# MuMuJun97/semantic_slam_mapping

Hardware: AMD Instinct MI355X
Metric: frames/sec semantic-mapping, 640x480 RGB-D (higher is better)
Workload: dtype u8; 1 GPU; configs[1]: synthetic 640x480 RGB-D + precomputed 12-class masks, 1k frames per GPU, ORB 1000 kp/frame, 5 ref frames, leaf 0.10 m; frames_per_gpu=1000, frames_all_gpus=1000, batch_frames=250, matcher_halo_frames=0, parallelism=single GPU

## Files before the change

### semantic_slam_mapping_amd/csrc/kernels_orb.hip

```cpp
#include "ssm_internal.h"
#include "../../include/ssm/fast_quick_core.h"
#include <cstdlib>
#include <type_traits>
#include <algorithm>
#include <cstring>
#include <vector>

#define WAVE 64

template <bool VEC>
__global__ void gray_kernel(const uint8_t* __restrict__ img, int W, int H, int stride0, uint8_t* __restrict__ pyr, int pyr_bytes)
{
    const int quads = stride0 >> 2;
    const int q = blockIdx.x * blockDim.x + threadIdx.x;
    if (q >= quads * H) return;
    const int y = q / quads, x = (q - y * quads) << 2;
    const uint8_t* src = img + (size_t)blockIdx.y * W * H * 3 + ((size_t)y * W + x) * 3;
    uint8_t* dst = pyr + (size_t)blockIdx.y * pyr_bytes + (size_t)y * stride0 + x;
    uint32_t out = 0;
    if (x >= W) { *reinterpret_cast<uint32_t*>(dst) = 0; return; }
    if (VEC) {
        const uint32_t* s = reinterpret_cast<const uint32_t*>(src);
        uint32_t a = s[0], b = s[1], c = s[2];
        uint32_t p0 = ((a & 255) * 1868 + ((a >> 8) & 255) * 9617 + ((a >> 16) & 255) * 4899 + 8192) >> 14;
// ... 694 lines not shown
        const int w0 = wsum[0], w1 = wsum[1], w2 = wsum[2];
        n = w0 + w1 + w2 + wsum[3];
        int base = (int)(incl - cnt) + (wv > 0 ? w0 : 0) + (wv > 1 ? w1 : 0) + (wv > 2 ? w2 : 0);
        const uint32_t ent = ((uint32_t)(tid >> 2) << 8) | (uint32_t)(32 * (tid & 3));
        while (m) { list[base++] = (uint16_t)(ent + (uint32_t)__builtin_ctz(m)); m &= m - 1u; }
    }
    __syncthreads();
    const int ix0 = X0 - xs0, iw = X1 - X0, iy0 = Y0 - ys0, ih = Y1 - Y0;
    for (int e0 = 0; e0 < n; e0 += 512) {
        const int m = min(n - e0, 512), H = (m + 1) >> 1;
        const bool act = wv * 64 < H;
        bool ka = false, kb = false; int ia = 0, ib = 0;
        if (act) {
            const int ea = tid, eb = H + tid;
            ia = list[e0 + min(ea, m - 1)]; ib = list[e0 + min(eb, m - 1)];
            const int sya = ia >> 8, sxa = ia & 255, syb = ib >> 8, sxb = ib & 255;
            const uint32_t S2 = fast_S2(&px[(sya + 3) * FT_PW + sxa + 4], &px[(syb + 3) * FT_PW + sxb + 4], FT_PW);
            const int Sa = (int)(S2 & 0xFFFFu), Sb = (int)(S2 >> 16);
            if (ea < H) sc[(sya + 1) * FT_SST + sxa + 1] = (uint8_t)Sa;
            if (eb < m) sc[(syb + 1) * FT_SST + sxb + 1] = (uint8_t)Sb;
            ka = ea < H && Sa > min_th && (unsigned)(sxa - ix0) < (unsigned)iw && (unsigned)(sya - iy0) < (unsigned)ih;
            kb = eb < m && Sb > min_th && (unsigned)(sxb - ix0) < (unsigned)iw && (unsigned)(syb - iy0) < (unsigned)ih;
        }
        __syncthreads();
        if (act) {
            const unsigned long long ba = __ballot(ka), bb = __ballot(kb);
            const int ca = __popcll(ba), cb = __popcll(bb);
            if (ca + cb) {
                int base = 0;
                if (lane == 0) base = atomicAdd(&nsurv, ca + cb);
                base = __shfl(base, 0, 64);
                const unsigned long long below = (1ull << lane) - 1ull;
                if (ka) list[base + __popcll(ba & below)] = (uint16_t)ia;
                if (kb) list[base + ca + __popcll(bb & below)] = (uint16_t)ib;
            }
        }
    }
    __syncthreads();
    const int n2 = nsurv;
    cand_t* out = cand + (size_t)frame * g.cand_total + L.cand_off;
    int32_t* nc = ncand + frame * g.nlevels + l;
    for (int e0 = 0; e0 < n2; e0 += 256) {
        if (e0 + wv * 64 >= n2) continue;
        const int e = e0 + tid;
        bool keep = false; int S = 0, sx = 0, sy = 0;
        if (e < n2) {
            const int i = list[e]; sy = i >> 8; sx = i & 255;
            const uint8_t* q = &sc[(sy + 1) * FT_SST + sx + 1];
            S = q[0];
            const int cx = cellx[sx + 1], cy = celly[sy + 1];
            const bool xl = cellx[sx] == cx, xr = cellx[sx + 2] == cx, yu = celly[sy] == cy, yd = celly[sy + 2] == cy;
            int nb = 0;
            if (yu) { nb = max(nb, (int)q[-FT_SST]); if (xl) nb = max(nb, (int)q[-FT_SST-1]); if (xr) nb = max(nb, (int)q[-FT_SST+1]); }
            if (yd) { nb = max(nb, (int)q[FT_SST]);  if (xl) nb = max(nb, (int)q[FT_SST-1]);  if (xr) nb = max(nb, (int)q[FT_SST+1]); }
            if (xl) nb = max(nb, (int)q[-1]);
            if (xr) nb = max(nb, (int)q[1]);
            keep = nb < S;
        }
        const unsigned long long bal = __ballot(keep);
        if (bal) {
            int base = 0;
            if (lane == 0) base = atomicAdd(&nstage, __popcll(bal));
            base = __shfl(base, 0, 64);
            if (keep) {
                const int k = base + __popcll(bal & ((1ull << lane) - 1ull));
                const int gx = xs0 + sx, gy = ys0 + sy;
                const int cj = cellx[sx + 1], ci = celly[sy + 1];
                atomicMax(&lmax[((ci - cy0) & 7) * 8 + ((cj - cx0) & 7)], S);
                cand_t c;
                c.x = (uint32_t)(gx - L.minBX) | ((uint32_t)(gy - L.minBY) << 12) | ((uint32_t)(S - 1) << 24);
                c.y = ((uint32_t)(ci * L.nCols + cj) << 14) | ((uint32_t)(gy - L.minBY - ci * L.hCell) << 7) | (uint32_t)(gx - L.minBX - cj * L.wCell);
                if (k < stage_cap) stage[k] = c;
                else { const int kg = atomicAdd(nc, 1); if (kg < L.cand_cap) out[kg] = c; }
            }
        }
    }
    __syncthreads();
    const int ns = min(nstage, stage_cap);
    if (tid == 0 && ns) gbase = atomicAdd(nc, ns);
    __syncthreads();
    for (int k = tid; k < ns; k += 256) if (gbase + k < L.cand_cap) out[gbase + k] = stage[k];
    if (tid < 64 && lmax[tid] > 0) {
        const int ci = cy0 + (tid >> 3), cj = cx0 + (tid & 7);
        atomicMax(&cellmax[(size_t)frame * g.cells_total + L.cell_off + ci * L.nCols + cj], lmax[tid]);
    }
}
__global__ void __launch_bounds__(256, 8)
fast_kernel(const uint8_t* __restrict__ pyr, OrbGeom g, cand_t* __restrict__ cand, int32_t* __restrict__ ncand, int32_t* __restrict__ cellmax, int stage_cap, int nframes)
{
    const int frame = blockIdx.x, tile_id = blockIdx.y;
    if (frame >= nframes) return;
    fast_tile<1>(frame, tile_id, pyr, g, cand, ncand, cellmax, stage_cap);
}
__global__ void __launch_bounds__(256)
fast_need_kernel(OrbGeom g, const int32_t* __restrict__ cellmax, int nframes, int32_t* __restrict__ work)
{
    const int i = blockIdx.x * blockDim.x + threadIdx.x;
    const int frame = i % ((nframes + 7) & ~7), tile_id = i / ((nframes + 7) & ~7);
    bool need = false;
    if (frame < nframes && tile_id < g.ftiles_total) {
        int l = 0;
        while (l + 1 < g.nlevels && tile_id >= g.L[l+1].ftile_off) l++;
        const LevelGeom& L = g.L[l];
        const int t = tile_id - L.ftile_off;
        const int trow = L.ftiles_x == 1 ? t : (int)__umulhi((uint32_t)t, L.fmulTX);
        int X0, X1, Y0, Y1;
        ftile_rect(L, t - trow * L.ftiles_x, trow, X0, X1, Y0, Y1);
        const int cx0 = (int)__umulhi((uint32_t)(X0 - L.minBX - 3), L.mulW), cy0 = (int)__umulhi((uint32_t)(Y0 - L.minBY - 3), L.mulH);
        const int cx1 = min((int)__umulhi((uint32_t)(X1 - 1 - L.minBX - 3), L.mulW), L.nCols - 1), cy1 = min((int)__umulhi((uint32_t)(Y1 - 1 - L.minBY - 3), L.mulH), L.nRows - 1);
        const int32_t* cm = cellmax + (size_t)frame * g.cells_total + L.cell_off;
        for (int ci = cy0; ci <= cy1 && !need; ci++) for (int cj = cx0; cj <= cx1; cj++) if (cm[ci * L.nCols + cj] <= g.ini_th) { need = true; break; }
    }
    const unsigned long long bal = __ballot(need);
    if (bal) {
        const int lane = threadIdx.x & 63;
        int base = 0;
        if (lane == 0) base = atomicAdd(work - 1, __popcll(bal));
        base = __shfl(base, 0, 64);
        if (need) work[base + __popcll(bal & ((1ull << lane) - 1ull))] = (tile_id << 16) | frame;
    }
}
__global__ void __launch_bounds__(256)
fast_retry_kernel(const uint8_t* __restrict__ pyr, OrbGeom g, cand_t* __restrict__ cand, int32_t* __restrict__ ncand, int32_t* __restrict__ cellmax, int stage_cap,
                  const int32_t* __restrict__ work)
{
    const int nwork = work[-1];
    for (int i = blockIdx.x; i < nwork; i += gridDim.x) {
        const int item = work[i];
        fast_tile<2>(item & 65535, item >> 16, pyr, g, cand, ncand, cellmax, stage_cap);
        __syncthreads();
    }
}
size_t k_fast_cellmax_ints(int nframes, const OrbGeom& g) { return (size_t)nframes * (g.cells_total + g.ftiles_total) + 16; }
size_t k_fast_ncand_pad(int nframes, const OrbGeom& g) { return ((size_t)nframes * g.nlevels + 63) & ~(size_t)63; }
hipError_t k_fast(int n, const OrbGeom& g, const uint8_t* pyr, cand_t* cand, int32_t* ncand, int32_t* cellmax, hipStream_t s)
{
    hipError_t e;
    const ptrdiff_t gap = cellmax - ncand;
    if (gap >= (ptrdiff_t)n * g.nlevels && gap <= (ptrdiff_t)1 << 24) e = hipMemsetAsync(ncand, 0, sizeof(int32_t) * (((size_t)gap + (size_t)n * g.cells_total + 4 + 3) & ~(size_t)3), s);
    else { e = hipMemsetAsync(ncand, 0, sizeof(int32_t) * n * g.nlevels, s); if (e == hipSuccess) e = hipMemsetAsync(cellmax, 0, sizeof(int32_t) * ((size_t)n * g.cells_total + 4), s); }
    if (e != hipSuccess) return e;
    static const int stage_cap = [] { const char* e = getenv("SSM_FAST_STAGE_CAP"); const int v = e ? atoi(e) : FT_STAGE; return v < 0 ? 0 : (v > FT_STAGE ? FT_STAGE : v); }();
    int32_t* work = cellmax + (size_t)n * g.cells_total + 4;
    const int n8 = (n + 7) & ~7;
    fast_kernel<<<dim3(n8, g.ftiles_total), 256, 0, s>>>(pyr, g, cand, ncand, cellmax, stage_cap, n);
    fast_need_kernel<<<(n8 * g.ftiles_total + 255) / 256, 256, 0, s>>>(g, cellmax, n, work);
    const int pairs = n * g.ftiles_total;
    fast_retry_kernel<<<pairs < 4096 ? pairs : 4096, 256, 0, s>>>(pyr, g, cand, ncand, cellmax, stage_cap, work);
    return hipGetLastError();
}

struct QNode { short x0, y0, x1, y1; };
#define DROPPED 0xFFFF
#define OT_KCAP 2048
#define OT_T 256
#define OT_UN 4
__device__ __forceinline__ uint32_t block_excl_scan_u32(uint32_t v, uint32_t* sw, uint32_t& total)
{
    const uint32_t inc = wave_incl_scan_u32(v);
    const int lane = threadIdx.x & 63, w = threadIdx.x >> 6;
    if (lane == 63) sw[w] = inc;
    __syncthreads();
    uint32_t base = 0, tot = 0;
#pragma unroll
    for (int k = 0; k < OT_T / 64; k++) { const uint32_t x = sw[k]; tot += x; if (k < w) base += x; }
    __syncthreads();
    total = tot;
    return inc - v + base;
}
#ifdef SSM_OT_PROF
__device__ unsigned long long ot_prof[8][8];
#define OTP_T0 long long otp_ = clock64();
#define OTP(k) { const long long n_ = clock64(); if (threadIdx.x == 0) atomicAdd(&ot_prof[blockIdx.y & 7][k], (unsigned long long)(n_ - otp_)); otp_ = n_; }
#define OTP_CNT(k) { if (threadIdx.x == 0) atomicAdd(&ot_prof[blockIdx.y & 7][k], 1ull); }
#else
#define OTP_T0
#define OTP(k)
#define OTP_CNT(k)
#endif
template <int NODES>
__global__ void __launch_bounds__(OT_T, NODES == 256 ? 8 : 1)
octree_kernel(OrbGeom g, const cand_t* __restrict__ cand, const int32_t* __restrict__ ncand, const int32_t* __restrict__ cellmax,
              uint16_t* __restrict__ node_of, uint32_t* __restrict__ sel, int32_t* __restrict__ nsel, int32_t* __restrict__ status)
{
    __shared__ QNode    nd[2][NODES];
    __shared__ uint32_t cnt[2][NODES];
    __shared__ uint32_t sq[2][NODES];
    __shared__ __attribute__((aligned(8))) uint32_t cc[NODES][4];
    __shared__ short    newpos[NODES];
    __shared__ __attribute__((aligned(8))) short childpos[NODES][4];
    __shared__ short    order[NODES];
    unsigned long long* best = reinterpret_cast<unsigned long long*>(&cc[0][0]);
    __shared__ uint16_t lnof[OT_KCAP];
    __shared__ uint16_t cumn[NODES];
    __shared__ uint32_t sscan[OT_T / 64];
    __shared__ int sL, sFinish, sMode, sErr, sValid, sFirst;
    const int l = blockIdx.y, f = blockIdx.x, tid = threadIdx.x;
    OTP_T0
    const LevelGeom& L = g.L[l];
    const int N = L.nfeat;
    int nc = ncand[f * g.nlevels + l];
    if (nc > L.cand_cap) { nc = L.cand_cap; if (tid == 0) atomicOr(status, 1); }
    const cand_t* gkeys = cand + (size_t)f * g.cand_total + L.cand_off;
    uint16_t* gnof = node_of + (size_t)f * g.cand_total + L.cand_off;
    const bool in_lds = nc <= OT_KCAP;
    constexpr int KPT = OT_KCAP / OT_T;
    uint32_t kxr[KPT];
#pragma unroll
    for (int u = 0; u < KPT; u++) kxr[u] = 0u;
#define KEY(i) (gkeys[i])
#define KEYX(i) (gkeys[i].x)
#define NOF(i) (in_lds ? lnof[i] : gnof[i])
#define SETNOF(i, v) do { if (in_lds) lnof[i] = (uint16_t)(v); else gnof[i] = (uint16_t)(v); } while (0)
    uint32_t* out = sel + (size_t)f * g.sel_total + L.sel_off;
    if (nc == 0) { if (tid == 0) nsel[f * g.nlevels + l] = 0; return; }
    const int nIni = L.nIni; const float hX = L.hX;
    for (int i = tid; i < nIni; i += OT_T) {
        QNode q; q.x0 = (short)(int)(hX * (float)i); q.y0 = 0; q.x1 = (short)(int)(hX * (float)(i + 1)); q.y1 = (short)(L.maxBY - L.minBY);
        nd[0][i] = q; cnt[0][i] = 0; sq[0][i] = i;
    }
    if (tid == 0) { sErr = 0; sValid = 0; }
    __syncthreads();
    const int32_t* cm = cellmax + (size_t)f * g.cells_total + L.cell_off;
    int nvalid = 0;
    auto init_trip = [&](auto lds_tag, int i0, cand_t (&k)[OT_UN]) {
        constexpr bool in_lds = decltype(lds_tag)::value;
        int cmv[OT_UN];
#pragma unroll
        for (int u = 0; u < OT_UN; u++) { const int i = i0 + u * OT_T; k[u] = i < nc ? KEY(i) : make_uint2(0u, 0u); }
#pragma unroll
        for (int u = 0; u < OT_UN; u++) cmv[u] = i0 + u * OT_T < nc ? cm[k[u].y >> 14] : 0;
#pragma unroll
        for (int u = 0; u < OT_UN; u++) {
            const int i = i0 + u * OT_T;
            if (i >= nc) continue;
            const int S = (int)(k[u].x >> 24) + 1;
            const int th = cmv[u] > g.ini_th ? g.ini_th : g.min_th;
            if (S <= th) { SETNOF(i, DROPPED); continue; }
            const int x = k[u].x & 4095;
            int b = (int)((float)x / hX); b = min(b, nIni - 1);
            SETNOF(i, b); atomicAdd(&cnt[0][b], 1u); nvalid++;
        }
    };
    if (in_lds) {
#pragma unroll
        for (int t = 0; t < KPT / OT_UN; t++) {
            const int i0 = tid + t * OT_UN * OT_T;
            if (i0 < nc) { cand_t k[OT_UN]; init_trip(std::true_type{}, i0, k); for (int u = 0; u < OT_UN; u++) kxr[t * OT_UN + u] = k[u].x; }
        }
    } else {
        for (int i0 = tid; i0 < nc; i0 += OT_UN * OT_T) { cand_t k[OT_UN]; init_trip(std::false_type{}, i0, k); }
    }
    if (nvalid) atomicAdd(&sValid, nvalid);
    __syncthreads();
    if (sValid == 0) { if (tid == 0) nsel[f * g.nlevels + l] = 0; return; }
    if (tid == 0) {
        int pos = 0;
        for (int i = 0; i < nIni; i++) {
            if (cnt[0][i] == 0) { newpos[i] = -1; continue; }
            nd[1][pos] = nd[0][i]; cnt[1][pos] = cnt[0][i]; sq[1][pos] = sq[0][i]; newpos[i] = (short)pos; pos++;
        }
        sL = pos; sFinish = 0; sMode = 0;
    }
    __syncthreads();
    if (in_lds) { for (int i = tid; i < nc; i += OT_T) { const int o = lnof[i]; if (o != DROPPED) lnof[i] = (uint16_t)newpos[o]; } }
    else        { for (int i = tid; i < nc; i += OT_T) { const int o = gnof[i]; if (o != DROPPED) gnof[i] = (uint16_t)newpos[o]; } }
    int cur = 1;
    __syncthreads();
    OTP(0)
    while (!sFinish) {
        const int Lsz = sL;
        QNode* cn = nd[cur]; uint32_t* ccnt = cnt[cur]; uint32_t* csq = sq[cur];
        QNode* nn = nd[cur ^ 1]; uint32_t* ncnt = cnt[cur ^ 1]; uint32_t* nsq = sq[cur ^ 1];
        unsigned long long* okey = reinterpret_cast<unsigned long long*>(&childpos[0][0]);
        for (int i = tid; i < Lsz; i += OT_T) {
            cc[i][0] = cc[i][1] = cc[i][2] = cc[i][3] = 0;
            const uint32_t ci = ccnt[i];
            okey[i] = ci > 1 ? (((unsigned long long)ci << 32) | csq[i]) + 1ull : 0ull;
        }
        __syncthreads();
        auto count_trip = [&](auto lds_tag, int i0, const uint32_t (&kx)[OT_UN]) {
            constexpr bool in_lds = decltype(lds_tag)::value;
            int ni[OT_UN]; uint32_t cn_[OT_UN]; QNode q[OT_UN];
#pragma unroll
            for (int u = 0; u < OT_UN; u++) { const int i = i0 + u * OT_T; ni[u] = i < nc ? (int)NOF(i) : DROPPED; }
#pragma unroll
            for (int u = 0; u < OT_UN; u++) cn_[u] = ni[u] != DROPPED ? ccnt[ni[u]] : 0u;
#pragma unroll
            for (int u = 0; u < OT_UN; u++) q[u] = cn[ni[u] != DROPPED ? ni[u] : 0];
#pragma unroll
            for (int u = 0; u < OT_UN; u++) {
                if (cn_[u] > 1) {
                    const int x = kx[u] & 4095, y = (kx[u] >> 12) & 4095;
                    const int mx = q[u].x0 + ((q[u].x1 - q[u].x0 + 1) >> 1), my = q[u].y0 + ((q[u].y1 - q[u].y0 + 1) >> 1);
                    const int qd = (x < mx) ? (y < my ? 0 : 2) : (y < my ? 1 : 3);
                    atomicAdd(&cc[ni[u]][qd], 1u);
                }
            }
        };
        if (in_lds) {
#pragma unroll
            for (int t = 0; t < KPT / OT_UN; t++) {
                const int i0 = tid + t * OT_UN * OT_T;
                if (i0 < nc) { uint32_t kx[OT_UN]; for (int u = 0; u < OT_UN; u++) kx[u] = kxr[t * OT_UN + u]; count_trip(std::true_type{}, i0, kx); }
            }
        } else {
            for (int i0 = tid; i0 < nc; i0 += OT_UN * OT_T) {
                uint32_t kx[OT_UN];
#pragma unroll
                for (int u = 0; u < OT_UN; u++) { const int i = i0 + u * OT_T; kx[u] = i < nc ? KEYX(i) : 0u; }
                count_trip(std::false_type{}, i0, kx);
            }
        }
        OTP(1)
        if (sMode == 1) for (int i = tid; i < Lsz; i += OT_T) {
            const unsigned long long ki = okey[i];
            if (ki) {
                int r = 0;
#pragma unroll 8
                for (int j = 0; j < Lsz; j++) r += okey[j] > ki ? 1 : 0;
                order[r] = (short)i;
            }
        }
        __syncthreads();
        OTP(2)
        #define EMIT_CHILDREN(i, e, cb)                                                                     \
            {   const QNode q = cn[i];                                                                      \
                const int mx = q.x0 + ((q.x1 - q.x0 + 1) >> 1), my = q.y0 + ((q.y1 - q.y0 + 1) >> 1);       \
                int p_ = (cb);                                                                              \
                for (int qd = 3; qd >= 0; qd--) {                                                           \
                    const uint32_t c = cc[i][qd];                                                           \
                    if (c == 0) { childpos[i][qd] = -1; continue; }                                         \
                    if (p_ < NODES) {                                                                       \
                        QNode ch;                                                                           \
                        ch.x0 = (qd & 1) ? (short)mx : q.x0; ch.x1 = (qd & 1) ? q.x1 : (short)mx;           \
                        ch.y0 = (qd & 2) ? (short)my : q.y0; ch.y1 = (qd & 2) ? q.y1 : (short)my;           \
                        nn[p_] = ch; ncnt[p_] = c; nsq[p_] = 4u * (uint32_t)(e) + (uint32_t)qd;             \
                        childpos[i][qd] = (short)p_;                                                        \
                    } else childpos[i][qd] = 0;                                                             \
                    p_++;                                                                                   \
                }                                                                                           \
            }
        constexpr int IPT = NODES > OT_T ? NODES / OT_T : 1;
        const int mode = sMode;
        uint32_t aloc[IPT], bloc[IPT], asum = 0, bsum = 0;
#pragma unroll
        for (int k = 0; k < IPT; k++) {
            const int i = tid * IPT + k;
            aloc[k] = 0; bloc[k] = 0;
            if (i < Lsz) {
                if (ccnt[i] > 1) {
                    aloc[k] = 1u;
                    for (int qd = 0; qd < 4; qd++) { const uint32_t c = cc[i][qd]; bloc[k] += (c > 0 ? 1u : 0u) + (c > 1 ? 0x10000u : 0u); }
                } else aloc[k] = 0x10000u;
            }
            asum += aloc[k]; bsum += bloc[k];
        }
        uint32_t aT, bT;
        uint32_t aP = block_excl_scan_u32(asum, sscan, aT);
        uint32_t bP = block_excl_scan_u32(bsum, sscan, bT);
        const int E = (int)(aT & 0xFFFFu);
        int pos_total;
        if (mode == 0) {
            const int totalCh = (int)(bT & 0xFFFFu);
            pos_total = totalCh + (int)(aT >> 16);
#pragma unroll
            for (int k = 0; k < IPT; k++) {
                const int i = tid * IPT + k;
                if (i < Lsz) {
                    if (aloc[k] & 1u) {
                        const int e = (int)(aP & 0xFFFFu), cb = totalCh - (int)((bP & 0xFFFFu) + (bloc[k] & 0xFFFFu));
                        EMIT_CHILDREN(i, e, cb); newpos[i] = -2;
                    } else {
                        const int p_ = totalCh + (int)(aP >> 16);
                        if (p_ < NODES) { nn[p_] = cn[i]; ncnt[p_] = ccnt[i]; nsq[p_] = csq[i]; newpos[i] = (short)p_; } else newpos[i] = 0;
                    }
                }
                aP += aloc[k]; bP += bloc[k];
            }
            if (tid == 0) {
                if (pos_total >= N || pos_total == Lsz) sFinish = 1;
                else if (pos_total + 3 * (int)(bT >> 16) > N) sMode = 1;
            }
        } else {
            if (tid == 0) sFirst = E - 1;
            uint32_t nloc[IPT], nsum = 0;
#pragma unroll
            for (int k = 0; k < IPT; k++) {
                const int r = tid * IPT + k;
                nloc[k] = 0;
                if (r < E) { const int i = order[r]; for (int qd = 0; qd < 4; qd++) nloc[k] += cc[i][qd] > 0 ? 1u : 0u; }
                nsum += nloc[k];
            }
            uint32_t nT;
            uint32_t nP = block_excl_scan_u32(nsum, sscan, nT);
#pragma unroll
            for (int k = 0; k < IPT; k++) {
                const int r = tid * IPT + k;
                nP += nloc[k];
                if (r < E) {
                    cumn[r] = (uint16_t)nP;
                    if (Lsz + (int)nP - (r + 1) >= N) atomicMin(&sFirst, r);
                }
            }
            for (int i = tid; i < Lsz; i += OT_T) newpos[i] = 0;
            __syncthreads();
            const int nsplit = E > 0 ? sFirst + 1 : 0, totalCh = nsplit > 0 ? (int)cumn[nsplit - 1] : 0;
            pos_total = totalCh + Lsz - nsplit;
#pragma unroll
            for (int k = 0; k < IPT; k++) {
                const int r = tid * IPT + k;
                if (r < nsplit) { const int i = order[r]; EMIT_CHILDREN(i, r, totalCh - (int)cumn[r]); newpos[i] = -2; }
            }
            __syncthreads();
            uint32_t kloc[IPT], ksum = 0;
#pragma unroll
            for (int k = 0; k < IPT; k++) { const int i = tid * IPT + k; kloc[k] = (i < Lsz && newpos[i] != -2) ? 1u : 0u; ksum += kloc[k]; }
            uint32_t kT;
            uint32_t kP = block_excl_scan_u32(ksum, sscan, kT);
#pragma unroll
            for (int k = 0; k < IPT; k++) {
                const int i = tid * IPT + k;
                if (kloc[k]) {
                    const int p_ = totalCh + (int)kP;
                    if (p_ < NODES) { nn[p_] = cn[i]; ncnt[p_] = ccnt[i]; nsq[p_] = csq[i]; newpos[i] = (short)p_; } else newpos[i] = 0;
                }
                kP += kloc[k];
            }
            if (tid == 0 && (pos_total >= N || pos_total == Lsz)) sFinish = 1;
        }
        #undef EMIT_CHILDREN
        if (tid == 0) {
            if (pos_total > NODES) { sErr = 1; sFinish = 1; pos_total = NODES; }
            sL = pos_total;
        }
        __syncthreads();
        OTP(3)
        auto relabel_trip = [&](auto lds_tag, int i0, const uint32_t (&kx)[OT_UN]) {
            constexpr bool in_lds = decltype(lds_tag)::value;
            int ni[OT_UN]; int np_[OT_UN]; QNode q[OT_UN];
#pragma unroll
            for (int u = 0; u < OT_UN; u++) { const int i = i0 + u * OT_T; ni[u] = i < nc ? (int)NOF(i) : DROPPED; }
#pragma unroll
            for (int u = 0; u < OT_UN; u++) { const int n_ = ni[u] != DROPPED ? ni[u] : 0; np_[u] = newpos[n_]; q[u] = cn[n_]; }
#pragma unroll
            for (int u = 0; u < OT_UN; u++) {
                if (ni[u] == DROPPED) continue;
                const int i = i0 + u * OT_T;
                if (np_[u] == -2) {
                    const int x = kx[u] & 4095, y = (kx[u] >> 12) & 4095;
                    const int mx = q[u].x0 + ((q[u].x1 - q[u].x0 + 1) >> 1), my = q[u].y0 + ((q[u].y1 - q[u].y0 + 1) >> 1);
                    const int qd = (x < mx) ? (y < my ? 0 : 2) : (y < my ? 1 : 3);
                    SETNOF(i, childpos[ni[u]][qd]);
                } else SETNOF(i, np_[u]);
            }
        };
        if (in_lds) {
#pragma unroll
            for (int t = 0; t < KPT / OT_UN; t++) {
                const int i0 = tid + t * OT_UN * OT_T;
                if (i0 < nc) { uint32_t kx[OT_UN]; for (int u = 0; u < OT_UN; u++) kx[u] = kxr[t * OT_UN + u]; relabel_trip(std::true_type{}, i0, kx); }
            }
        } else {
            for (int i0 = tid; i0 < nc; i0 += OT_UN * OT_T) {
                uint32_t kx[OT_UN];
#pragma unroll
                for (int u = 0; u < OT_UN; u++) { const int i = i0 + u * OT_T; kx[u] = i < nc ? KEYX(i) : 0u; }
                relabel_trip(std::false_type{}, i0, kx);
            }
        }
        cur ^= 1;
        __syncthreads();
        OTP(4) OTP_CNT(7)
    }
    const int Lf = sL;
    if (sErr && tid == 0) atomicOr(status, 2);
    for (int i = tid; i < Lf; i += OT_T) best[i] = 0ull;
    __syncthreads();
    for (int i0 = tid; i0 < nc; i0 += OT_UN * OT_T) {
        int ni[OT_UN]; cand_t k[OT_UN];
#pragma unroll
        for (int u = 0; u < OT_UN; u++) { const int i = i0 + u * OT_T; ni[u] = i < nc ? (in_lds ? (int)lnof[i] : (int)gnof[i]) : DROPPED; k[u] = i < nc ? KEY(i) : make_uint2(0u, 0u); }
#pragma unroll
        for (int u = 0; u < OT_UN; u++) {
            if (ni[u] == DROPPED) continue;
            const unsigned long long v = ((unsigned long long)(k[u].x >> 24) << 56) | ((unsigned long long)(0xFFFFFFFFu - k[u].y) << 24) | (k[u].x & 0xFFFFFFu);
            atomicMax(&best[ni[u]], v);
        }
    }
    __syncthreads();
    for (int i = tid; i < Lf && i < L.sel_cap; i += OT_T) {
        const unsigned long long v = best[i];
        const uint32_t x = (uint32_t)(v & 4095) + L.minBX, y = (uint32_t)((v >> 12) & 4095) + L.minBY, s = (uint32_t)(v >> 56);
        out[i] = x | (y << 12) | (s << 24);
    }
    if (tid == 0) { nsel[f * g.nlevels + l] = min(Lf, L.sel_cap); if (Lf > L.sel_cap) atomicOr(status, 4); }
    OTP(5)
}
#ifdef SSM_OT_PROF
extern "C" void ssm_debug_octree_prof(void)
{
    unsigned long long h[8][8];
    if (hipMemcpyFromSymbol(h, HIP_SYMBOL(ot_prof), sizeof(h)) != hipSuccess) return;
    for (int l = 0; l < 8; l++) fprintf(stderr, "octree level %d: init %llu count-sweep %llu order %llu rebuild %llu relabel %llu best %llu | passes %llu\n", l, h[l][0], h[l][1], h[l][2], h[l][3], h[l][4], h[l][5], h[l][7]);
    for (auto& r_ : h) for (auto& v_ : r_) v_ = 0;
    (void)hipMemcpyToSymbol(HIP_SYMBOL(ot_prof), h, sizeof(h));
}
#endif
hipError_t k_octree(int n, const OrbGeom& g, const cand_t* cand, const int32_t* ncand, const int32_t* cellmax, uint16_t* node_of,
                    uint32_t* sel, int32_t* nsel, int32_t* status, hipStream_t s)
{
    int need = 0;
    for (int l = 0; l < g.nlevels; l++) need = need > g.L[l].nfeat + 3 ? need : g.L[l].nfeat + 3;
    for (int l = 0; l < g.nlevels; l++) need = need > 4 * g.L[l].nIni + 8 ? need : 4 * g.L[l].nIni + 8;
    if (need <= 256 - 8) octree_kernel<256><<<dim3(n, g.nlevels), OT_T, 0, s>>>(g, cand, ncand, cellmax, node_of, sel, nsel, status);
    else if (need <= 512 - 8) octree_kernel<512><<<dim3(n, g.nlevels), OT_T, 0, s>>>(g, cand, ncand, cellmax, node_of, sel, nsel, status);
    else                 octree_kernel<1024><<<dim3(n, g.nlevels), OT_T, 0, s>>>(g, cand, ncand, cellmax, node_of, sel, nsel, status);
    return hipGetLastError();
}

__device__ __forceinline__ float fast_atan2_deg(float y, float x)
{
    const float p1 = 0.9997878412794807f * (float)(180 / 3.14159265358979323846);
    const float p3 = -0.3258083974640975f * (float)(180 / 3.14159265358979323846);
    const float p5 = 0.1555786518463281f * (float)(180 / 3.14159265358979323846);
    const float p7 = -0.04432655554792128f * (float)(180 / 3.14159265358979323846);
    const float ax = fabsf(x), ay = fabsf(y);
    float a, c, c2;
    if (ax >= ay) { c = ay / (ax + (float)2.2204460492503131e-16); c2 = c * c; a = (((p7 * c2 + p5) * c2 + p3) * c2 + p1) * c; }
    else          { c = ax / (ay + (float)2.2204460492503131e-16); c2 = c * c; a = 90.f - (((p7 * c2 + p5) * c2 + p3) * c2 + p1) * c; }
    if (x < 0) a = 180.f - a;
    if (y < 0) a = 360.f - a;
    return a;
}
__device__ __forceinline__ void contract_sincos(float angle_rad, float* s, float* c)
{
    const double PIO2_HI = 1.57079632673412561417e+00, PIO2_LO = 6.07710050650619224932e-11;
    const double x = (double)angle_rad;
    const double kd = rint(x * 0.63661977236758134308);
    const int k = (int)kd;
    const double r = (x - kd * PIO2_HI) - kd * PIO2_LO;
    const double r2 = r * r;
    double ps = -1.0 / 1307674368000.0;
    ps = ps * r2 + 1.0 / 6227020800.0;
    ps = ps * r2 - 1.0 / 39916800.0;
    ps = ps * r2 + 1.0 / 362880.0;
    ps = ps * r2 - 1.0 / 5040.0;
    ps = ps * r2 + 1.0 / 120.0;
    ps = ps * r2 - 1.0 / 6.0;
    const double sn = r + r * (r2 * ps);
    double pc = 1.0 / 20922789888000.0;
    pc = pc * r2 - 1.0 / 87178291200.0;
    pc = pc * r2 + 1.0 / 479001600.0;
    pc = pc * r2 - 1.0 / 3628800.0;
    pc = pc * r2 + 1.0 / 40320.0;
    pc = pc * r2 - 1.0 / 720.0;
    pc = pc * r2 + 1.0 / 24.0;
    pc = pc * r2 - 0.5;
    const double cs = 1.0 + r2 * pc;
    double S, C;
    switch (k & 3) { case 0: S = sn; C = cs; break; case 1: S = cs; C = -sn; break; case 2: S = -sn; C = -cs; break; default: S = -cs; C = sn; break; }
    *s = (float)S; *c = (float)C;
}
__device__ __forceinline__ int wave_total(int v) { return __builtin_amdgcn_readlane((int)wave_incl_scan_u32((uint32_t)v), 63); }
struct KpAux { int32_t m10, m01; float sn, cs; };
#define DP_ROWS_O 31
#define DP_QW_O 3
#define DP_ROWS_B 37
#define DP_QW_B 4
__device__ __forceinline__ bool kp_slot(const OrbGeom& g, const int32_t* __restrict__ ns, int slot, int& l, int& oidx)
{
    if (slot >= g.sel_total) return false;
    l = 0;
    while (l + 1 < g.nlevels && slot >= g.L[l+1].sel_off) l++;
    const int i = slot - g.L[l].sel_off;
    if (i >= ns[l]) return false;
    oidx = i;
    for (int k = 0; k < l; k++) oidx += ns[k];
    return true;
}
struct KpRec { uint32_t off; uint32_t stride_level; int32_t oidx; uint32_t pk; };
__global__ void __launch_bounds__(256)
kp_prepare_kernel(OrbGeom g, const uint32_t* __restrict__ sel, const int32_t* __restrict__ nsel, KpRec* __restrict__ recs, int32_t* __restrict__ nkp)
{
    const int f = blockIdx.y, slot = blockIdx.x * 256 + threadIdx.x;
    const int32_t* ns = nsel + f * g.nlevels;
    if (slot == 0) { int t = 0; for (int l = 0; l < g.nlevels; l++) t += ns[l]; nkp[f] = t; }
    if (slot >= g.sel_total) return;
    int l, oidx;
    KpRec r; r.off = 0; r.stride_level = 0; r.oidx = -1; r.pk = 0;
    if (kp_slot(g, ns, slot, l, oidx)) {
        const LevelGeom& L = g.L[l];
        r.pk = sel[(size_t)f * g.sel_total + slot];
        const int x = r.pk & 4095, y = (r.pk >> 12) & 4095;
        r.off = (uint32_t)(L.img_off + y * L.stride + x); r.stride_level = (uint32_t)L.stride | ((uint32_t)l << 16); r.oidx = oidx;
    }
    recs[(size_t)f * g.sel_total + slot] = r;
}
#define OR_KPW 4
__device__ __forceinline__ uint32_t udot4(uint32_t a, uint32_t b, uint32_t acc) { return __builtin_amdgcn_udot4(a, b, acc, false); }
__global__ void __launch_bounds__(256)
orient_kernel(OrbGeom g, unsigned long long umax_pack, const uint8_t* __restrict__ pyr, const KpRec* __restrict__ recs, KpAux* __restrict__ aux, int nframes)
{
    const int lane = threadIdx.x & 63, wv = threadIdx.x >> 6, f = blockIdx.x;
    const int slot0 = (blockIdx.y * 4 + wv) * OR_KPW;
    if (f >= nframes || slot0 >= g.sel_total) return;
    const int r = lane >> 1, left = !(lane & 1);
    const int v = r <= 2 * SSM_HALF_PATCH ? r - SSM_HALF_PATCH : 0;
    const int d = r <= 2 * SSM_HALF_PATCH ? (int)((umax_pack >> (4 * (v < 0 ? -v : v))) & 15ull) : -1;
    uint32_t M[4];
#pragma unroll
    for (int j = 0; j < 4; j++) {
        uint32_t m = 0;
#pragma unroll
        for (int k = 0; k < 4; k++) {
            const int kk = 4 * j + k;
            const bool keep = left ? (kk >= 16 - d && d > 0) : (kk <= d);
            m |= keep ? (0xFFu << (8 * k)) : 0u;
        }
        M[j] = m;
    }
    const int koff = left ? -16 : 0;
    const uint8_t* fr = pyr + (size_t)f * g.pyr_bytes;
    uint4 px[OR_KPW]; bool ok[OR_KPW]; KpRec rec[OR_KPW];
#pragma unroll
    for (int q = 0; q < OR_KPW; q++) rec[q] = recs[(size_t)f * g.sel_total + min(slot0 + q, g.sel_total - 1)];
#pragma unroll
    for (int q = 0; q < OR_KPW; q++) {
        ok[q] = slot0 + q < g.sel_total && rec[q].oidx >= 0;
        const uint8_t* p = ok[q] ? fr + rec[q].off + v * (int)(rec[q].stride_level & 0xFFFFu) + koff : fr;
        uint4 t; __builtin_memcpy(&t, p, 16);
        px[q] = t;
    }
#pragma unroll
    for (int q = 0; q < OR_KPW; q++) {
        if (!ok[q]) continue;
        const uint32_t a0 = px[q].x & M[0], a1 = px[q].y & M[1], a2 = px[q].z & M[2], a3 = px[q].w & M[3];
        uint32_t si = udot4(a0, 0x01010101u, 0u); si = udot4(a1, 0x01010101u, si); si = udot4(a2, 0x01010101u, si); si = udot4(a3, 0x01010101u, si);
        uint32_t sk = udot4(a0, 0x03020100u, 0u); sk = udot4(a1, 0x07060504u, sk); sk = udot4(a2, 0x0B0A0908u, sk); sk = udot4(a3, 0x0F0E0D0Cu, sk);
        const int sui = (int)sk - (left ? 16 * (int)si : 0);
        const int m10 = wave_total(sui), m01 = wave_total(v * (int)si);
        if (lane == 0) { KpAux a; a.m10 = m10; a.m01 = m01; a.sn = 0.f; a.cs = 0.f; aux[(size_t)f * g.sel_total + slot0 + q] = a; }
    }
}
__global__ void __launch_bounds__(256)
angle_kernel(OrbGeom g, const KpRec* __restrict__ recs, const uint16_t* __restrict__ depth, ssm_camera cam,
             KpAux* __restrict__ aux, ssm_keypoint* __restrict__ kps, float* __restrict__ pos3d)
{
    const int f = blockIdx.y, slot = blockIdx.x * 256 + threadIdx.x;
    if (slot >= g.sel_total) return;
    const KpRec rec = recs[(size_t)f * g.sel_total + slot];
    if (rec.oidx < 0) return;
    const int l = (int)(rec.stride_level >> 16), oidx = rec.oidx;
    const LevelGeom& L = g.L[l];
    const uint32_t pk = rec.pk;
    const int x = pk & 4095, y = (pk >> 12) & 4095, score = pk >> 24;
    KpAux a = aux[(size_t)f * g.sel_total + slot];
// ... 129 lines not shown
```

Before: 191,500 frames/s.

## Keep more octree node ids in LDS with u8 labels and fewer barriers

For the 256-node octree variant, per-candidate node labels become uint8 in LDS, which raises the in-LDS candidate capacity from 2048 to 4096 so larger levels avoid global node_of traffic. Other changes: the two block scans are fused into one with a single barrier, the per-pass clearing of cc and okey moves to the end of the previous pass, and the relabel sweep is skipped when no initial node is empty. Keys beyond the register cache are reloaded from global memory on each pass. The risks are more LDS use, lower occupancy and subtle correctness issues around the uint8 drop sentinel and the moved initialisation.

```diff
diff --git a/semantic_slam_mapping_amd/csrc/kernels_orb.hip b/semantic_slam_mapping_amd/csrc/kernels_orb.hip
--- a/semantic_slam_mapping_amd/csrc/kernels_orb.hip
+++ b/semantic_slam_mapping_amd/csrc/kernels_orb.hip
@@ -870,7 +870,8 @@
 
 struct QNode { short x0, y0, x1, y1; };
 #define DROPPED 0xFFFF
-#define OT_KCAP 2048
+template <int NODES> struct OtIds { typedef uint16_t lds_t; static constexpr int KCAP = 2048; };
+template <> struct OtIds<256> { typedef uint8_t lds_t; static constexpr int KCAP = 4096; };
 #define OT_T 256
 #define OT_UN 4
 __device__ __forceinline__ uint32_t block_excl_scan_u32(uint32_t v, uint32_t* sw, uint32_t& total)
@@ -882,25 +883,40 @@
     uint32_t base = 0, tot = 0;
 #pragma unroll
     for (int k = 0; k < OT_T / 64; k++) { const uint32_t x = sw[k]; tot += x; if (k < w) base += x; }
-    __syncthreads();
     total = tot;
     return inc - v + base;
+}
+__device__ __forceinline__ void block_excl_scan2_u32(uint32_t a, uint32_t b, uint32_t* sw, uint32_t& pa, uint32_t& pb, uint32_t& ta, uint32_t& tb)
+{
+    const uint32_t ia = wave_incl_scan_u32(a), ib = wave_incl_scan_u32(b);
+    const int lane = threadIdx.x & 63, w = threadIdx.x >> 6;
+    if (lane == 63) { sw[w] = ia; sw[OT_T / 64 + w] = ib; }
+    __syncthreads();
+    uint32_t ba = 0, bb = 0, sa = 0, sb = 0;
+#pragma unroll
+    for (int k = 0; k < OT_T / 64; k++) { const uint32_t x = sw[k], y = sw[OT_T / 64 + k]; sa += x; sb += y; if (k < w) { ba += x; bb += y; } }
+    ta = sa; tb = sb;
+    pa = ia - a + ba; pb = ib - b + bb;
 }
 #ifdef SSM_OT_PROF
 __device__ unsigned long long ot_prof[8][8];
 #define OTP_T0 long long otp_ = clock64();
 #define OTP(k) { const long long n_ = clock64(); if (threadIdx.x == 0) atomicAdd(&ot_prof[blockIdx.y & 7][k], (unsigned long long)(n_ - otp_)); otp_ = n_; }
-#define OTP_CNT(k) { if (threadIdx.x == 0) atomicAdd(&ot_prof[blockIdx.y & 7][k], 1ull); }
+#define OTP_CNT(k) OTP_ADD(k, 1)
+#define OTP_ADD(k, v) { if (threadIdx.x == 0) atomicAdd(&ot_prof[blockIdx.y & 7][k], (unsigned long long)(v)); }
 #else
 #define OTP_T0
 #define OTP(k)
 #define OTP_CNT(k)
+#define OTP_ADD(k, v)
 #endif
 template <int NODES>
 __global__ void __launch_bounds__(OT_T, NODES == 256 ? 8 : 1)
 octree_kernel(OrbGeom g, const cand_t* __restrict__ cand, const int32_t* __restrict__ ncand, const int32_t* __restrict__ cellmax,
               uint16_t* __restrict__ node_of, uint32_t* __restrict__ sel, int32_t* __restrict__ nsel, int32_t* __restrict__ status)
 {
+    typedef typename OtIds<NODES>::lds_t lnof_t;
+    constexpr int KCAP = OtIds<NODES>::KCAP, LDROP = (lnof_t)~(lnof_t)0;
     __shared__ QNode    nd[2][NODES];
     __shared__ uint32_t cnt[2][NODES];
     __shared__ uint32_t sq[2][NODES];
@@ -909,9 +925,9 @@
     __shared__ __attribute__((aligned(8))) short childpos[NODES][4];
     __shared__ short    order[NODES];
     unsigned long long* best = reinterpret_cast<unsigned long long*>(&cc[0][0]);
-    __shared__ uint16_t lnof[OT_KCAP];
+    __shared__ lnof_t   lnof[KCAP];
     __shared__ uint16_t cumn[NODES];
-    __shared__ uint32_t sscan[OT_T / 64];
+    __shared__ uint32_t sscan[3 * (OT_T / 64)];
     __shared__ int sL, sFinish, sMode, sErr, sValid, sFirst;
     const int l = blockIdx.y, f = blockIdx.x, tid = threadIdx.x;
     OTP_T0
@@ -921,35 +937,39 @@
     if (nc > L.cand_cap) { nc = L.cand_cap; if (tid == 0) atomicOr(status, 1); }
     const cand_t* gkeys = cand + (size_t)f * g.cand_total + L.cand_off;
     uint16_t* gnof = node_of + (size_t)f * g.cand_total + L.cand_off;
-    const bool in_lds = nc <= OT_KCAP;
-    constexpr int KPT = OT_KCAP / OT_T;
+    const bool in_lds = nc <= KCAP;
+    OTP_ADD(6, nc)
+    constexpr int KPT = 2048 / OT_T, TRIPS = KCAP / (OT_UN * OT_T);
     uint32_t kxr[KPT];
 #pragma unroll
     for (int u = 0; u < KPT; u++) kxr[u] = 0u;
 #define KEY(i) (gkeys[i])
 #define KEYX(i) (gkeys[i].x)
-#define NOF(i) (in_lds ? lnof[i] : gnof[i])
-#define SETNOF(i, v) do { if (in_lds) lnof[i] = (uint16_t)(v); else gnof[i] = (uint16_t)(v); } while (0)
+#define NOF(i) (in_lds ? (int)lnof[i] : (int)gnof[i])
+#define NDROP (in_lds ? LDROP : DROPPED)
+#define SETNOF(i, v) do { if (in_lds) lnof[i] = (lnof_t)(v); else gnof[i] = (uint16_t)(v); } while (0)
     uint32_t* out = sel + (size_t)f * g.sel_total + L.sel_off;
     if (nc == 0) { if (tid == 0) nsel[f * g.nlevels + l] = 0; return; }
     const int nIni = L.nIni; const float hX = L.hX;
     for (int i = tid; i < nIni; i += OT_T) {
         QNode q; q.x0 = (short)(int)(hX * (float)i); q.y0 = 0; q.x1 = (short)(int)(hX * (float)(i + 1)); q.y1 = (short)(L.maxBY - L.minBY);
         nd[0][i] = q; cnt[0][i] = 0; sq[0][i] = i;
+        cc[i][0] = cc[i][1] = cc[i][2] = cc[i][3] = 0;
     }
     if (tid == 0) { sErr = 0; sValid = 0; }
     __syncthreads();
     const int32_t* cm = cellmax + (size_t)f * g.cells_total + L.cell_off;
     int nvalid = 0;
-    auto init_trip = [&](auto lds_tag, int i0, cand_t (&k)[OT_UN]) {
+    auto init_trip = [&](auto lds_tag, int i0, auto& k) {
         constexpr bool in_lds = decltype(lds_tag)::value;
-        int cmv[OT_UN];
-#pragma unroll
-        for (int u = 0; u < OT_UN; u++) { const int i = i0 + u * OT_T; k[u] = i < nc ? KEY(i) : make_uint2(0u, 0u); }
-#pragma unroll
-        for (int u = 0; u < OT_UN; u++) cmv[u] = i0 + u * OT_T < nc ? cm[k[u].y >> 14] : 0;
-#pragma unroll
-        for (int u = 0; u < OT_UN; u++) {
+        constexpr int NK = (int)(sizeof(k) / sizeof(k[0]));
+        int cmv[NK];
+#pragma unroll
+        for (int u = 0; u < NK; u++) { const int i = i0 + u * OT_T; k[u] = i < nc ? KEY(i) : make_uint2(0u, 0u); }
+#pragma unroll
+        for (int u = 0; u < NK; u++) cmv[u] = i0 + u * OT_T < nc ? cm[k[u].y >> 14] : 0;
+#pragma unroll
+        for (int u = 0; u < NK; u++) {
             const int i = i0 + u * OT_T;
             if (i >= nc) continue;
             const int S = (int)(k[u].x >> 24) + 1;
@@ -957,14 +977,14 @@
             if (S <= th) { SETNOF(i, DROPPED); continue; }
             const int x = k[u].x & 4095;
             int b = (int)((float)x / hX); b = min(b, nIni - 1);
-            SETNOF(i, b); atomicAdd(&cnt[0][b], 1u); nvalid++;
+            SETNOF(i, b); if (nIni > 1) atomicAdd(&cnt[0][b], 1u); nvalid++;
         }
     };
     if (in_lds) {
 #pragma unroll
-        for (int t = 0; t < KPT / OT_UN; t++) {
-            const int i0 = tid + t * OT_UN * OT_T;
-            if (i0 < nc) { cand_t k[OT_UN]; init_trip(std::true_type{}, i0, k); for (int u = 0; u < OT_UN; u++) kxr[t * OT_UN + u] = k[u].x; }
+        for (int t = 0; t < TRIPS / 2; t++) {
+            const int i0 = tid + t * KPT * OT_T;
+            if (i0 < nc) { cand_t k[KPT]; init_trip(std::true_type{}, i0, k); if (t == 0) for (int u = 0; u < KPT; u++) kxr[u] = k[u].x; }
         }
     } else {
         for (int i0 = tid; i0 < nc; i0 += OT_UN * OT_T) { cand_t k[OT_UN]; init_trip(std::false_type{}, i0, k); }
@@ -975,14 +995,17 @@
     if (tid == 0) {
         int pos = 0;
         for (int i = 0; i < nIni; i++) {
-            if (cnt[0][i] == 0) { newpos[i] = -1; continue; }
-            nd[1][pos] = nd[0][i]; cnt[1][pos] = cnt[0][i]; sq[1][pos] = sq[0][i]; newpos[i] = (short)pos; pos++;
+            const uint32_t ci = nIni > 1 ? cnt[0][i] : (uint32_t)sValid;
+            if (ci == 0) { newpos[i] = -1; continue; }
+            nd[1][pos] = nd[0][i]; cnt[1][pos] = ci; sq[1][pos] = sq[0][i]; newpos[i] = (short)pos; pos++;
         }
         sL = pos; sFinish = 0; sMode = 0;
     }
     __syncthreads();
-    if (in_lds) { for (int i = tid; i < nc; i += OT_T) { const int o = lnof[i]; if (o != DROPPED) lnof[i] = (uint16_t)newpos[o]; } }
-    else        { for (int i = tid; i < nc; i += OT_T) { const int o = gnof[i]; if (o != DROPPED) gnof[i] = (uint16_t)newpos[o]; } }
+    if (sL != nIni) {
+        if (in_lds) { for (int i = tid; i < nc; i += OT_T) { const int o = lnof[i]; if (o != LDROP) lnof[i] = (lnof_t)newpos[o]; } }
+        else        { for (int i = tid; i < nc; i += OT_T) { const int o = gnof[i]; if (o != DROPPED) gnof[i] = (uint16_t)newpos[o]; } }
+    }
     int cur = 1;
     __syncthreads();
     OTP(0)
@@ -991,21 +1014,15 @@
         QNode* cn = nd[cur]; uint32_t* ccnt = cnt[cur]; uint32_t* csq = sq[cur];
         QNode* nn = nd[cur ^ 1]; uint32_t* ncnt = cnt[cur ^ 1]; uint32_t* nsq = sq[cur ^ 1];
         unsigned long long* okey = reinterpret_cast<unsigned long long*>(&childpos[0][0]);
-        for (int i = tid; i < Lsz; i += OT_T) {
-            cc[i][0] = cc[i][1] = cc[i][2] = cc[i][3] = 0;
-            const uint32_t ci = ccnt[i];
-            okey[i] = ci > 1 ? (((unsigned long long)ci << 32) | csq[i]) + 1ull : 0ull;
-        }
-        __syncthreads();
         auto count_trip = [&](auto lds_tag, int i0, const uint32_t (&kx)[OT_UN]) {
             constexpr bool in_lds = decltype(lds_tag)::value;
             int ni[OT_UN]; uint32_t cn_[OT_UN]; QNode q[OT_UN];
 #pragma unroll
-            for (int u = 0; u < OT_UN; u++) { const int i = i0 + u * OT_T; ni[u] = i < nc ? (int)NOF(i) : DROPPED; }
-#pragma unroll
-            for (int u = 0; u < OT_UN; u++) cn_[u] = ni[u] != DROPPED ? ccnt[ni[u]] : 0u;
-#pragma unroll
-            for (int u = 0; u < OT_UN; u++) q[u] = cn[ni[u] != DROPPED ? ni[u] : 0];
+            for (int u = 0; u < OT_UN; u++) { const int i = i0 + u * OT_T; ni[u] = i < nc ? NOF(i) : NDROP; }
+#pragma unroll
+            for (int u = 0; u < OT_UN; u++) cn_[u] = ni[u] != NDROP ? ccnt[ni[u]] : 0u;
+#pragma unroll
+            for (int u = 0; u < OT_UN; u++) q[u] = cn[ni[u] != NDROP ? ni[u] : 0];
 #pragma unroll
             for (int u = 0; u < OT_UN; u++) {
                 if (cn_[u] > 1) {
@@ -1018,9 +1035,15 @@
         };
         if (in_lds) {
 #pragma unroll
-            for (int t = 0; t < KPT / OT_UN; t++) {
+            for (int t = 0; t < TRIPS; t++) {
                 const int i0 = tid + t * OT_UN * OT_T;
-                if (i0 < nc) { uint32_t kx[OT_UN]; for (int u = 0; u < OT_UN; u++) kx[u] = kxr[t * OT_UN + u]; count_trip(std::true_type{}, i0, kx); }
+                if (i0 < nc) {
+                    uint32_t kx[OT_UN];
+                    int j0 = i0;
+                    if (t >= KPT / OT_UN) asm volatile("" : "+v"(j0));
+                    for (int u = 0; u < OT_UN; u++) kx[u] = t < KPT / OT_UN ? kxr[(t * OT_UN + u) % KPT] : (i0 + u * OT_T < nc ? KEYX(j0 + u * OT_T) : 0u);
+                    count_trip(std::true_type{}, i0, kx);
+                }
             }
         } else {
             for (int i0 = tid; i0 < nc; i0 += OT_UN * OT_T) {
@@ -1074,9 +1097,8 @@
             }
             asum += aloc[k]; bsum += bloc[k];
         }
-        uint32_t aT, bT;
-        uint32_t aP = block_excl_scan_u32(asum, sscan, aT);
-        uint32_t bP = block_excl_scan_u32(bsum, sscan, bT);
+        uint32_t aT, bT, aP, bP;
+        block_excl_scan2_u32(asum, bsum, sscan, aP, bP, aT, bT);
         const int E = (int)(aT & 0xFFFFu);
         int pos_total;
         if (mode == 0) {
@@ -1111,7 +1133,7 @@
                 nsum += nloc[k];
             }
             uint32_t nT;
-            uint32_t nP = block_excl_scan_u32(nsum, sscan, nT);
+            uint32_t nP = block_excl_scan_u32(nsum, sscan + 2 * (OT_T / 64), nT);
 #pragma unroll
             for (int k = 0; k < IPT; k++) {
                 const int r = tid * IPT + k;
@@ -1154,16 +1176,18 @@
         }
         __syncthreads();
         OTP(3)
+        const int Lnext = sL;
+        for (int i = tid; i < Lnext; i += OT_T) cc[i][0] = cc[i][1] = cc[i][2] = cc[i][3] = 0;
         auto relabel_trip = [&](auto lds_tag, int i0, const uint32_t (&kx)[OT_UN]) {
             constexpr bool in_lds = decltype(lds_tag)::value;
             int ni[OT_UN]; int np_[OT_UN]; QNode q[OT_UN];
 #pragma unroll
-            for (int u = 0; u < OT_UN; u++) { const int i = i0 + u * OT_T; ni[u] = i < nc ? (int)NOF(i) : DROPPED; }
-#pragma unroll
-            for (int u = 0; u < OT_UN; u++) { const int n_ = ni[u] != DROPPED ? ni[u] : 0; np_[u] = newpos[n_]; q[u] = cn[n_]; }
+            for (int u = 0; u < OT_UN; u++) { const int i = i0 + u * OT_T; ni[u] = i < nc ? NOF(i) : NDROP; }
+#pragma unroll
+            for (int u = 0; u < OT_UN; u++) { const int n_ = ni[u] != NDROP ? ni[u] : 0; np_[u] = newpos[n_]; q[u] = cn[n_]; }
 #pragma unroll
             for (int u = 0; u < OT_UN; u++) {
-                if (ni[u] == DROPPED) continue;
+                if (ni[u] == NDROP) continue;
                 const int i = i0 + u * OT_T;
                 if (np_[u] == -2) {
                     const int x = kx[u] & 4095, y = (kx[u] >> 12) & 4095;
@@ -1175,9 +1199,15 @@
         };
         if (in_lds) {
 #pragma unroll
-            for (int t = 0; t < KPT / OT_UN; t++) {
+            for (int t = 0; t < TRIPS; t++) {
                 const int i0 = tid + t * OT_UN * OT_T;
-                if (i0 < nc) { uint32_t kx[OT_UN]; for (int u = 0; u < OT_UN; u++) kx[u] = kxr[t * OT_UN + u]; relabel_trip(std::true_type{}, i0, kx); }
+                if (i0 < nc) {
+                    uint32_t kx[OT_UN];
+                    int j0 = i0;
+                    if (t >= KPT / OT_UN) asm volatile("" : "+v"(j0));
+                    for (int u = 0; u < OT_UN; u++) kx[u] = t < KPT / OT_UN ? kxr[(t * OT_UN + u) % KPT] : (i0 + u * OT_T < nc ? KEYX(j0 + u * OT_T) : 0u);
+                    relabel_trip(std::true_type{}, i0, kx);
+                }
             }
         } else {
             for (int i0 = tid; i0 < nc; i0 += OT_UN * OT_T) {
@@ -1189,6 +1219,13 @@
         }
         cur ^= 1;
         __syncthreads();
+        if (sMode == 1 && !sFinish) {
+            for (int i = tid; i < Lnext; i += OT_T) {
+                const uint32_t ci = ncnt[i];
+                okey[i] = ci > 1 ? (((unsigned long long)ci << 32) | nsq[i]) + 1ull : 0ull;
+            }
+            __syncthreads();
+        }
         OTP(4) OTP_CNT(7)
     }
     const int Lf = sL;
@@ -1198,7 +1235,7 @@
     for (int i0 = tid; i0 < nc; i0 += OT_UN * OT_T) {
         int ni[OT_UN]; cand_t k[OT_UN];
 #pragma unroll
-        for (int u = 0; u < OT_UN; u++) { const int i = i0 + u * OT_T; ni[u] = i < nc ? (in_lds ? (int)lnof[i] : (int)gnof[i]) : DROPPED; k[u] = i < nc ? KEY(i) : make_uint2(0u, 0u); }
+        for (int u = 0; u < OT_UN; u++) { const int i = i0 + u * OT_T; ni[u] = i < nc ? (in_lds ? (lnof[i] == LDROP ? DROPPED : (int)lnof[i]) : (int)gnof[i]) : DROPPED; k[u] = i < nc ? KEY(i) : make_uint2(0u, 0u); }
 #pragma unroll
         for (int u = 0; u < OT_UN; u++) {
             if (ni[u] == DROPPED) continue;
@@ -1220,7 +1257,7 @@
 {
     unsigned long long h[8][8];
     if (hipMemcpyFromSymbol(h, HIP_SYMBOL(ot_prof), sizeof(h)) != hipSuccess) return;
-    for (int l = 0; l < 8; l++) fprintf(stderr, "octree level %d: init %llu count-sweep %llu order %llu rebuild %llu relabel %llu best %llu | passes %llu\n", l, h[l][0], h[l][1], h[l][2], h[l][3], h[l][4], h[l][5], h[l][7]);
+    for (int l = 0; l < 8; l++) fprintf(stderr, "octree level %d: init %llu count-sweep %llu order %llu rebuild %llu relabel %llu best %llu | keys %llu passes %llu\n", l, h[l][0], h[l][1], h[l][2], h[l][3], h[l][4], h[l][5], h[l][6], h[l][7]);
     for (auto& r_ : h) for (auto& v_ : r_) v_ = 0;
     (void)hipMemcpyToSymbol(HIP_SYMBOL(ot_prof), h, sizeof(h));
 }
```

Result: no change. 192,900 frames/s, median of 6 (+0.7%).
